# meijieru/AtomNAS

Hardware: AMD Instinct MI355X
Metric: images/sec (whole node) AtomNAS-C supernet 224x224 bs256/GPU (higher is better)
Workload: dtype bf16; 1 GPU; atomnas_c_supernet full training step (fwd + CE-smooth/L2/L1 + bwd + grad all-reduce + RMSprop + EMA), 224x224; per_gpu_batch=256, global_batch=256, parallelism=dp1, hip_graph=True

## Files before the change

### atomnas_amd/csrc/optim.hip

```cpp
#include "common.h"

namespace atomnas {

enum { HYP_LR = 0, HYP_RHO = 1, HYP_EMA_DECAY = 2, HYP_GRAD_SCALE = 3 };

enum { GUARD_OK = 0, GUARD_SCALE = 1, GUARD_NORM = 2, GUARD_COEF = 3, GUARD_SKIPPED = 4, GUARD_CLIPPED = 5 };

template <bool GUARDED>
__global__ __launch_bounds__(256) void k_rmsprop_ema(float* __restrict__ p, const float* __restrict__ g, float* __restrict__ sq,
                                                     float* __restrict__ buf, float* __restrict__ ema,
                                                     const float* __restrict__ wd_chunk, long n, const float* __restrict__ hyper,
                                                     float alpha, float one_minus_alpha, float eps, int eps_inside_sqrt,
                                                     float momentum, float* __restrict__ l2_part, const float* __restrict__ guard) {
#pragma clang fp contract(off)
  __shared__ float s_part[4];
  const float lr = hyper[HYP_LR], d = hyper[HYP_EMA_DECAY], gs = GUARDED ? guard[GUARD_SCALE] : hyper[HYP_GRAD_SCALE];
  const bool dropped = GUARDED && guard[GUARD_OK] == 0.f;
  const long nchunks = (n + 255) / 256;
  float l2acc = 0.f;
  for (long ch = blockIdx.x; ch < nchunks; ch += gridDim.x) {
    const long i = ch * 256 + threadIdx.x;
    if (i >= n) continue;
    const float wd = wd_chunk ? wd_chunk[ch] : 0.f;
    float pv = p[i];
// ... 122 lines not shown
}

constexpr int GUARD_UNROLL = 4;
constexpr int GUARD_SWEEP = 256 * GUARD_UNROLL;
constexpr int GUARD_MAX_BLOCKS = 1024;

__global__ __launch_bounds__(256) void k_grad_sumsq(const float* __restrict__ g, long n, float* __restrict__ part) {
#pragma clang fp contract(off)
  __shared__ float s_part[4];
  const long n4 = n >> 2;
  const f32x4* __restrict__ g4 = reinterpret_cast<const f32x4*>(g);
  float a[GUARD_UNROLL] = {0.f, 0.f, 0.f, 0.f};
  for (long base = (long)blockIdx.x * GUARD_SWEEP + threadIdx.x; base < n4; base += (long)gridDim.x * GUARD_SWEEP) {
    f32x4 v[GUARD_UNROLL];
#pragma unroll
    for (int u = 0; u < GUARD_UNROLL; ++u) {
      const long i = base + u * 256;
      v[u] = i < n4 ? g4[i] : f32x4{0.f, 0.f, 0.f, 0.f};
    }
#pragma unroll
    for (int u = 0; u < GUARD_UNROLL; ++u) a[u] = a[u] + ((v[u][0] * v[u][0] + v[u][1] * v[u][1]) + (v[u][2] * v[u][2] + v[u][3] * v[u][3]));
  }
  float acc = (a[0] + a[1]) + (a[2] + a[3]);
  const long t = n4 * 4 + threadIdx.x;
  if (blockIdx.x == 0 && threadIdx.x < 3 && t < n) acc = acc + g[t] * g[t];
  acc = wave_sum(acc);
  if ((threadIdx.x & 63) == 0) s_part[threadIdx.x >> 6] = acc;
  __syncthreads();
  if (threadIdx.x == 0) part[blockIdx.x] = ((s_part[0] + s_part[1]) + s_part[2]) + s_part[3];
}

__global__ __launch_bounds__(256) void k_guard_verdict(const float* __restrict__ part, int nparts, const float* __restrict__ hyper,
                                                       float max_norm, int skip_nonfinite, float* __restrict__ guard) {
#pragma clang fp contract(off)
  __shared__ float s_t[256];
  float a = 0.f;
  for (int i = threadIdx.x; i < nparts; i += 256) a += part[i];
  s_t[threadIdx.x] = a;
  __syncthreads();
  for (int o = 128; o > 0; o >>= 1) {
    if ((int)threadIdx.x < o) s_t[threadIdx.x] += s_t[threadIdx.x + o];
    __syncthreads();
  }
  if (threadIdx.x == 0) {
    const float sumsq = s_t[0], gs = hyper[HYP_GRAD_SCALE];
    const float norm = sqrtf(sumsq) * gs;
    const bool finite = isfinite(sumsq);
    float coef = 1.f;
    if (max_norm > 0.f && isfinite(max_norm) && isfinite(norm)) {
      const float c = max_norm / (norm + 1e-6f);
      coef = c < 1.f ? c : 1.f;
    }
    const bool ok = finite || !skip_nonfinite;
    guard[GUARD_OK] = ok ? 1.f : 0.f;
    guard[GUARD_SCALE] = gs * coef;
    guard[GUARD_NORM] = norm;
    guard[GUARD_COEF] = coef;
    int* cnt = reinterpret_cast<int*>(guard);
    if (!ok) cnt[GUARD_SKIPPED] = cnt[GUARD_SKIPPED] + 1;
    if (coef < 1.f) cnt[GUARD_CLIPPED] = cnt[GUARD_CLIPPED] + 1;
  }
}

__global__ __launch_bounds__(256) void k_guard_restore(float* __restrict__ dst, const float* __restrict__ src, long n,
                                                       const float* __restrict__ guard, int unconditional) {
  if (!unconditional && guard[GUARD_OK] != 0.f) return;
  const long n4 = n >> 2;
  f32x4* __restrict__ d4 = reinterpret_cast<f32x4*>(dst);
  const f32x4* __restrict__ s4 = reinterpret_cast<const f32x4*>(src);
  for (long i = (long)blockIdx.x * 256 + threadIdx.x; i < n4; i += (long)gridDim.x * 256) d4[i] = s4[i];
  const long t = n4 * 4 + threadIdx.x;
  if (blockIdx.x == 0 && threadIdx.x < 3 && t < n) dst[t] = src[t];
}

__global__ __launch_bounds__(256) void k_add_i64(long* __restrict__ p, long n, long v) {
  for (long i = (long)blockIdx.x * 256 + threadIdx.x; i < n; i += (long)gridDim.x * 256) p[i] += v;
}

struct PackJob {
  long src_off, dst_off;
  int rows, cols, src_ld, dst_ld, c_off, mode;
};

template <typename T>
__global__ __launch_bounds__(256) void k_pack(const float* __restrict__ arena, void* __restrict__ packbuf, const PackJob* __restrict__ jobs) {
  const PackJob jb = jobs[blockIdx.y];
  const long total = (long)jb.rows * jb.cols;
  const float* src = arena + jb.src_off;
  for (long i = (long)blockIdx.x * 256 + threadIdx.x; i < total; i += (long)gridDim.x * 256) {
    const int r = (int)(i / jb.cols), c = (int)(i % jb.cols);
    const float v = src[(long)r * jb.src_ld + c];
    if (jb.mode == 0) reinterpret_cast<T*>(packbuf)[jb.dst_off + (long)r * jb.dst_ld + jb.c_off + c] = from_f32<T>(v);
    else if (jb.mode == 1) reinterpret_cast<T*>(packbuf)[jb.dst_off + (long)(jb.c_off + c) * jb.dst_ld + r] = from_f32<T>(v);
    else reinterpret_cast<float*>(packbuf)[jb.dst_off + (long)c * jb.dst_ld + jb.c_off + r] = v;
  }
}

}

using namespace atomnas;

static int launch_rmsprop(const char* what, float* p, const float* g, float* sq, float* buf, float* ema, const float* wd_chunk, long n,
                          const float* hyper, double alpha, double eps, int eps_inside_sqrt, double momentum, float* l2_value, float* ws,
                          const float* guard, void* stream) {
  ATOMNAS_REQUIRE(p && g && sq && hyper && n > 0, "%s: bad arguments", what);
  ATOMNAS_REQUIRE(!l2_value || (ws && wd_chunk), "%s: the L2 value needs wd_chunk and a 4096-float workspace", what);
  ATOMNAS_REQUIRE(momentum >= 0.0 && alpha >= 0.0 && eps >= 0.0, "%s: bad hyper-parameters", what);
  ATOMNAS_REQUIRE((momentum > 0.0) == (buf != nullptr), "%s: momentum buffer must be given iff momentum > 0", what);
  long blocks = (n + 255) / 256;
  if (blocks > 4096) blocks = 4096;
  hipLaunchKernelGGL(guard ? k_rmsprop_ema<true> : k_rmsprop_ema<false>, dim3((unsigned)blocks), dim3(256), 0, (hipStream_t)stream, p, g, sq,
                     buf, ema, wd_chunk, n, hyper, (float)alpha, (float)(1.0 - alpha), (float)eps, eps_inside_sqrt, (float)momentum,
                     l2_value ? ws : nullptr, guard);
  if (l2_value)
    hipLaunchKernelGGL(k_sum_partials, dim3(1), dim3(256), 0, (hipStream_t)stream, ws, (int)blocks, 1.f, 0, l2_value);
  return check_launch(what);
}

extern "C" int atomnas_fused_rmsprop_ema(float* p, const float* g, float* sq, float* buf, float* ema, const float* wd_chunk, long n,
                                         const float* hyper, double alpha, double eps, int eps_inside_sqrt, double momentum,
                                         float* l2_value, float* ws, void* stream) {
  return launch_rmsprop("fused_rmsprop_ema", p, g, sq, buf, ema, wd_chunk, n, hyper, alpha, eps, eps_inside_sqrt, momentum, l2_value, ws,
                        nullptr, stream);
}

extern "C" int atomnas_fused_rmsprop_ema_guarded(float* p, const float* g, float* sq, float* buf, float* ema, const float* wd_chunk, long n,
                                                 const float* hyper, double alpha, double eps, int eps_inside_sqrt, double momentum,
                                                 float* l2_value, float* ws, const float* guard, void* stream) {
  ATOMNAS_REQUIRE(guard, "fused_rmsprop_ema_guarded: needs the guard vector");
  return launch_rmsprop("fused_rmsprop_ema_guarded", p, g, sq, buf, ema, wd_chunk, n, hyper, alpha, eps, eps_inside_sqrt, momentum, l2_value,
                        ws, guard, stream);
}

static int launch_sgd(const char* what, float* p, const float* g, float* buf, float* ema, const float* wd_chunk, long n, const float* hyper,
                      double momentum, int nesterov, float* l2_value, float* ws, const float* guard, void* stream) {
  ATOMNAS_REQUIRE(p && g && hyper && n > 0, "%s: bad arguments", what);
  ATOMNAS_REQUIRE(!l2_value || (ws && wd_chunk), "%s: the L2 value needs wd_chunk and a 4096-float workspace", what);
  ATOMNAS_REQUIRE(momentum >= 0.0, "%s: bad hyper-parameters", what);
  ATOMNAS_REQUIRE((momentum > 0.0) == (buf != nullptr), "%s: momentum buffer must be given iff momentum > 0", what);
  ATOMNAS_REQUIRE(!nesterov || momentum > 0.0, "%s: Nesterov momentum needs momentum > 0", what);
  long blocks = (n + 255) / 256;
  if (blocks > 4096) blocks = 4096;
  hipLaunchKernelGGL(guard ? k_sgd_ema<true> : k_sgd_ema<false>, dim3((unsigned)blocks), dim3(256), 0, (hipStream_t)stream, p, g, buf, ema,
                     wd_chunk, n, hyper, (float)momentum, nesterov, l2_value ? ws : nullptr, guard);
  if (l2_value)
    hipLaunchKernelGGL(k_sum_partials, dim3(1), dim3(256), 0, (hipStream_t)stream, ws, (int)blocks, 1.f, 0, l2_value);
  return check_launch(what);
}

extern "C" int atomnas_fused_sgd_ema(float* p, const float* g, float* buf, float* ema, const float* wd_chunk, long n, const float* hyper,
                                     double momentum, int nesterov, float* l2_value, float* ws, void* stream) {
  return launch_sgd("fused_sgd_ema", p, g, buf, ema, wd_chunk, n, hyper, momentum, nesterov, l2_value, ws, nullptr, stream);
}

extern "C" int atomnas_fused_sgd_ema_guarded(float* p, const float* g, float* buf, float* ema, const float* wd_chunk, long n,
                                             const float* hyper, double momentum, int nesterov, float* l2_value, float* ws,
                                             const float* guard, void* stream) {
  ATOMNAS_REQUIRE(guard, "fused_sgd_ema_guarded: needs the guard vector");
  return launch_sgd("fused_sgd_ema_guarded", p, g, buf, ema, wd_chunk, n, hyper, momentum, nesterov, l2_value, ws, guard, stream);
}

extern "C" int atomnas_grad_guard_ws_floats() { return GUARD_MAX_BLOCKS; }

extern "C" int atomnas_grad_guard(const float* g, long n, const float* hyper, float max_norm, int skip_nonfinite, float* ws, float* guard,
                                  void* stream) {
  ATOMNAS_REQUIRE(g && hyper && ws && guard && n > 0, "grad_guard: bad arguments");
  ATOMNAS_REQUIRE(((unsigned long long)g & 15ull) == 0, "grad_guard: needs a 16-byte aligned gradient arena");
  ATOMNAS_REQUIRE(!(max_norm != max_norm), "grad_guard: max_norm is NaN");
  long blocks = (n / 4 + GUARD_SWEEP - 1) / GUARD_SWEEP;
  if (blocks > GUARD_MAX_BLOCKS) blocks = GUARD_MAX_BLOCKS;
  if (blocks < 1) blocks = 1;
  hipLaunchKernelGGL(k_grad_sumsq, dim3((unsigned)blocks), dim3(256), 0, (hipStream_t)stream, g, n, ws);
  hipLaunchKernelGGL(k_guard_verdict, dim3(1), dim3(256), 0, (hipStream_t)stream, ws, (int)blocks, hyper, max_norm, skip_nonfinite, guard);
  return check_launch("grad_guard");
}

extern "C" int atomnas_guard_restore(float* dst, const float* src, long n, const float* guard, int unconditional, void* stream) {
  ATOMNAS_REQUIRE(dst && src && n > 0 && (guard || unconditional), "guard_restore: bad arguments");
  ATOMNAS_REQUIRE((((unsigned long long)dst | (unsigned long long)src) & 15ull) == 0, "guard_restore: needs 16-byte aligned pointers");
  long blocks = (n / 4 + 255) / 256;
  if (blocks > 2048) blocks = 2048;
  if (blocks < 1) blocks = 1;
  hipLaunchKernelGGL(k_guard_restore, dim3((unsigned)blocks), dim3(256), 0, (hipStream_t)stream, dst, src, n, guard, unconditional);
  return check_launch("guard_restore");
}

extern "C" int atomnas_vec_sum(const float* x, int n, float scale, float* out, void* stream) {
  ATOMNAS_REQUIRE(x && out && n > 0, "vec_sum: bad arguments");
  hipLaunchKernelGGL(k_sum_partials, dim3(1), dim3(256), 0, (hipStream_t)stream, x, n, scale, 0, out);
  return check_launch("vec_sum");
}

extern "C" int atomnas_ema_update(float* shadow, const float* x, long n, const float* hyper, void* stream) {
  ATOMNAS_REQUIRE(shadow && x && hyper && n > 0, "ema_update: bad arguments");
  long blocks = (n + 255) / 256;
  if (blocks > 2048) blocks = 2048;
  hipLaunchKernelGGL(k_ema<false>, dim3((unsigned)blocks), dim3(256), 0, (hipStream_t)stream, shadow, x, n, hyper, (const float*)nullptr);
  return check_launch("ema_update");
}

extern "C" int atomnas_ema_update_guarded(float* shadow, const float* x, long n, const float* hyper, const float* guard, void* stream) {
  ATOMNAS_REQUIRE(shadow && x && hyper && guard && n > 0, "ema_update_guarded: bad arguments");
  long blocks = (n + 255) / 256;
  if (blocks > 2048) blocks = 2048;
  hipLaunchKernelGGL(k_ema<true>, dim3((unsigned)blocks), dim3(256), 0, (hipStream_t)stream, shadow, x, n, hyper, guard);
  return check_launch("ema_update_guarded");
}

extern "C" int atomnas_scale_by(float* x, long n, const float* hyper, int idx, void* stream) {
  ATOMNAS_REQUIRE(x && hyper && n > 0 && idx >= 0 && idx < 4, "scale_by: bad arguments");
  long blocks = (n + 255) / 256;
  if (blocks > 2048) blocks = 2048;
  hipLaunchKernelGGL(k_scale_by, dim3((unsigned)blocks), dim3(256), 0, (hipStream_t)stream, x, n, hyper, idx);
  return check_launch("scale_by");
}

extern "C" int atomnas_accum_fold(float* acc, float* cur, const float* base, long n, int first, int last, float inv_count, void* stream) {
  ATOMNAS_REQUIRE(acc && cur && n > 0, "accum_fold: bad arguments");
  ATOMNAS_REQUIRE((((unsigned long long)acc | (unsigned long long)cur | (unsigned long long)base) & 15ull) == 0,
                  "accum_fold: needs 16-byte aligned pointers");
  long blocks = (n / 4 + 255) / 256;
  if (blocks > 2048) blocks = 2048;
  if (blocks < 1) blocks = 1;
  hipLaunchKernelGGL(k_accum_fold, dim3((unsigned)blocks), dim3(256), 0, (hipStream_t)stream, acc, cur, base, n, first, last, inv_count);
  return check_launch("accum_fold");
}

extern "C" int atomnas_zero(void* p, long bytes, void* stream) {
  ATOMNAS_REQUIRE(p && bytes > 0 && bytes % 4 == 0 && ((unsigned long long)p & 15ull) == 0, "zero: needs a 16-byte aligned pointer and whole words");
  const long n16 = bytes / 16;
  const int ntail = (int)((bytes % 16) / 4);
  long blocks = (n16 + 255) / 256;
  if (blocks > 4096) blocks = 4096;
  if (blocks < 1) blocks = 1;
  hipLaunchKernelGGL(k_zero, dim3((unsigned)blocks), dim3(256), 0, (hipStream_t)stream, (f32x4*)p, n16, (float*)p + n16 * 4, ntail);
  return check_launch("zero");
}

extern "C" int atomnas_add_i64(long* p, long n, long v, void* stream) {
  ATOMNAS_REQUIRE(p && n > 0, "add_i64: bad arguments");
  long blocks = (n + 255) / 256;
  if (blocks > 1024) blocks = 1024;
  hipLaunchKernelGGL(k_add_i64, dim3((unsigned)blocks), dim3(256), 0, (hipStream_t)stream, p, n, v);
  return check_launch("add_i64");
}

extern "C" int atomnas_pack_weights(const float* arena, void* packbuf, const void* jobs_dev, int njobs, int dtype, void* stream) {
  ATOMNAS_REQUIRE(arena && packbuf && jobs_dev && njobs > 0, "pack_weights: bad arguments");
  dim3 grid(32, njobs);
  hipStream_t st = (hipStream_t)stream;
  if (dtype == DT_F32) hipLaunchKernelGGL(k_pack<float>, grid, dim3(256), 0, st, arena, packbuf, (const PackJob*)jobs_dev);
  else hipLaunchKernelGGL(k_pack<bf16_t>, grid, dim3(256), 0, st, arena, packbuf, (const PackJob*)jobs_dev);
  return check_launch("pack_weights");
}

namespace atomnas {
struct RegJob {
  long off;
  int count;
  float coef;
};

__global__ __launch_bounds__(256) void k_reg_grad(const float* __restrict__ p, float* __restrict__ g, const RegJob* __restrict__ jobs,
                                                  int use_sign, const float* __restrict__ mult_ptr, const float* __restrict__ go_ptr) {
  const RegJob jb = jobs[blockIdx.y];
  float m = jb.coef;
  if (mult_ptr) m *= mult_ptr[0];
  if (go_ptr) m *= go_ptr[0];
  for (int i = blockIdx.x * 256 + threadIdx.x; i < jb.count; i += gridDim.x * 256) {
    const float v = p[jb.off + i];
    const float d = use_sign ? ((v > 0.f) ? 1.f : ((v < 0.f) ? -1.f : 0.f)) : v;
    g[jb.off + i] += m * d;
  }
}

__global__ __launch_bounds__(256) void k_reg_value(const float* __restrict__ p, const RegJob* __restrict__ jobs, int use_abs,
                                                   const float* __restrict__ mult_ptr, float post_scale, float* __restrict__ ws) {
  __shared__ float s_part[4];
  const RegJob jb = jobs[blockIdx.y];
  float acc = 0.f;
  for (int i = blockIdx.x * 256 + threadIdx.x; i < jb.count; i += gridDim.x * 256) {
    const float v = p[jb.off + i];
    acc += use_abs ? fabsf(v) : v * v;
  }
  acc = wave_sum(acc);
  if ((threadIdx.x & 63) == 0) s_part[threadIdx.x >> 6] = acc;
  __syncthreads();
  if (threadIdx.x == 0) {
    float m = jb.coef * post_scale;
    if (mult_ptr) m *= mult_ptr[0];
    ws[blockIdx.y * gridDim.x + blockIdx.x] = m * (((s_part[0] + s_part[1]) + s_part[2]) + s_part[3]);
  }
}

}

extern "C" int atomnas_reg_grad(const float* p, float* g, const void* jobs_dev, int njobs, int use_sign, const float* mult_ptr,
                                const float* grad_out_ptr, void* stream) {
  ATOMNAS_REQUIRE(p && g && jobs_dev && njobs > 0, "reg_grad: bad arguments");
  hipLaunchKernelGGL(atomnas::k_reg_grad, dim3(64, njobs), dim3(256), 0, (hipStream_t)stream, p, g, (const atomnas::RegJob*)jobs_dev,
                     use_sign, mult_ptr, grad_out_ptr);
  return atomnas::check_launch("reg_grad");
}

extern "C" int atomnas_reg_value(const float* p, const void* jobs_dev, int njobs, int use_abs, const float* mult_ptr,
                                 float post_scale, float* out, float* ws, void* stream) {
  ATOMNAS_REQUIRE(p && out && ws && jobs_dev && njobs > 0, "reg_value: bad arguments");
  hipLaunchKernelGGL(atomnas::k_reg_value, dim3(64, njobs), dim3(256), 0, (hipStream_t)stream, p, (const atomnas::RegJob*)jobs_dev,
                     use_abs, mult_ptr, post_scale, ws);
  hipLaunchKernelGGL(atomnas::k_sum_partials, dim3(1), dim3(256), 0, (hipStream_t)stream, ws, 64 * njobs, 1.f, 1, out);
  return atomnas::check_launch("reg_value");
}
```

### atomnas_amd/csrc/pwconv.hip

```cpp
#include "pwconv.h"

namespace atomnas {

template <typename T, int MODE, int NCG>
__global__ __launch_bounds__(256) void k_gemm_nt(Operand A, const T* __restrict__ Wp, int ldw, Epilogue ep, long M, int N, int K,
                                                 int Kpad) {
  using MM = Mma<T>;
  constexpr int E = MM::EPL;
  constexpr int KS = 4 * E;
  constexpr int SWD = 64 * NCG;
  extern __shared__ float s_stat[];

  const int tid = threadIdx.x;
  const int lane = tid & 63;
  const int wave = tid >> 6;
  const int q = lane >> 4, j = lane & 15;
  const int wrow = 16 * (j >> 2) + (j & 3);
  const bool do_stats = ep.stats != nullptr && ep.stat_mode != STAT_NONE;
  float* sw = s_stat + wave * 2 * SWD;

  if (do_stats) {
    for (int i = tid; i < 8 * SWD; i += 256) s_stat[i] = 0.f;
    __syncthreads();
  }
// ... 1881 lines not shown
  auto kern = k_gemm_nt_st<KSTEPS, EPK, Cfg::PD, BT, Cfg::WPE, 0, SH>;
  const size_t lds = (size_t)(SH ? 2 : 4) * BT * KSTEPS * 1024 +
                     (EPK == ST_FWD ? 0 : (size_t)4 * (16 + 64) * PB_RP * sizeof(bf16_t) + 4 * 128 * sizeof(float));
  const long waves = (long)num_cus() * resident_per_cu(kern, 256, lds) * 4;
  const long wchunks = SH ? (long)((nchunks + 3) / 4) * 4 : nchunks;
  long tiles_per_item = st_tiles_per_item(mtiles, wchunks, waves, min_tpi, 0);
  if (tiles_per_item > 4096) tiles_per_item = 4096;
  const long nrg = (mtiles + tiles_per_item - 1) / tiles_per_item;
  const long blocks = SH ? nrg * ((nchunks + 3) / 4) : (nrg * nchunks + 3) / 4;
  hipLaunchKernelGGL(kern, dim3((unsigned)blocks), dim3(256), lds, a.st, a.A, (const bf16_t*)a.Wp, a.ldw, ep, a.M, a.N, a.K, nchunks,
                     (int)tiles_per_item, (float*)nullptr);
  return check_launch("gemm_nt_st");
}
static int nt_st_launch(const NtStPlan& p, const NtArgs& a) {
  auto go = [&](auto ks, auto epk) {
    constexpr int KSTEPS = decltype(ks)::value, EPK = decltype(epk)::value;
    using Cfg = StCfg<KSTEPS, EPK>;
    const int nchunks = (a.N + 63) / 64;
    if (Cfg::SH && ((nchunks + 3) / 4 * 4 - nchunks) * 20 <= nchunks) return nt_st_launch_as<KSTEPS, EPK, Cfg::SH, Cfg::BT>(a);
    return nt_st_launch_as<KSTEPS, EPK, false, Cfg::BTP>(a);
  };
  auto kind = [&](auto ks) { return p.kind == ST_FWD ? go(ks, IC<ST_FWD>{}) : go(ks, IC<ST_MASK>{}); };
  return p.ksteps == 1 ? kind(IC<1>{}) : p.ksteps == 2 ? kind(IC<2>{}) : p.ksteps == 3 ? kind(IC<3>{}) : kind(IC<6>{});
}

struct NtSmallPlan { int kst, ntile; };
constexpr int SMALL_MAXN = 64, SMALL_MAXK = 64;
constexpr long SMALL_MINM = 65536;

static bool nt_small_plan(const NtArgs& a, NtSmallPlan& p) {
  if (a.N > SMALL_MAXN || a.K > SMALL_MAXK || a.M < SMALL_MINM) return false;
  p.kst = a.K <= 32 ? 1 : 2;
  p.ntile = (pw_env().small_narrow && !a.ep.out_f32 && a.N % 4 == 0) ? (a.N <= 16 ? 1 : a.N <= 32 ? 2 : 4) : 0;
  return true;
}
static int nt_small_launch(const NtSmallPlan& p, const NtArgs& a) {
  auto go = [&](auto mode, auto kst) {
    constexpr int MODE = decltype(mode)::value, KST = decltype(kst)::value;
    auto kern = p.ntile == 1 ? k_gemm_nt_small<MODE, KST, 1> : p.ntile == 2 ? k_gemm_nt_small<MODE, KST, 2>
              : p.ntile == 4 ? k_gemm_nt_small<MODE, KST, 4> : k_gemm_nt_small<MODE, KST, 0>;
    const size_t lds = a.stats ? (size_t)8 * 64 * sizeof(float) : 0;
    const long R = row_slots(kern, 256, lds, 1, (a.M + 63) / 64, stat_cap(a));
    hipLaunchKernelGGL(kern, dim3((unsigned)R), dim3(256), lds, a.st, a.A, (const bf16_t*)a.Wp, a.ldw, a.ep, a.M, a.N, a.K);
  };
  for_mode(a.mode, [&](auto mode) { p.kst == 1 ? go(mode, IC<1>{}) : go(mode, IC<2>{}); });
  return check_launch("gemm_nt_small");
}

struct NtWsPlan { int ncg, rt; };
constexpr int WS_MINK = 97;
constexpr long WS_MINM = 4096;
constexpr long WS_RT2_MINM = 100000;

static bool nt_ws_plan(const NtArgs& a, NtWsPlan& p) {
  if (a.K < WS_MINK || a.M < WS_MINM) return false;
  p.ncg = a.N > 64 ? 2 : 1;
  p.rt = (a.mode == PRO_BNBWD && a.M >= WS_RT2_MINM) ? 2 : 1;
  return true;
}
template <int MODE, int NCG, int RT>
static void nt_ws_launch_as(const NtArgs& a) {
  auto kern = k_gemm_nt_ws<MODE, NCG, RT>;
  const int ngroups = (a.N + 64 * NCG - 1) / (64 * NCG);
  const size_t lds = (size_t)2 * 64 * NCG * WS_WP * sizeof(bf16_t) + 2 * 3 * WS_KC * sizeof(float) +
                     (a.stats ? (size_t)8 * 64 * NCG * sizeof(float) : 0);
  const long R = row_slots(kern, 256, lds, ngroups, (a.M + 64 * RT - 1) / (64 * RT), stat_cap(a));
  const int wrows = (a.N + 63) / 64 * 64;
  hipLaunchKernelGGL(kern, dim3((unsigned)(R * ngroups)), dim3(256), lds, a.st, a.A, (const bf16_t*)a.Wp, a.ldw, wrows, a.ep, a.M, a.N, a.K);
}
static int nt_ws_launch(const NtWsPlan& p, const NtArgs& a) {
  for_mode(a.mode, [&](auto mode) {
    constexpr int MODE = decltype(mode)::value;
    if constexpr (MODE == PRO_BNBWD) {
      if (p.rt == 2) return p.ncg == 2 ? nt_ws_launch_as<MODE, 2, 2>(a) : nt_ws_launch_as<MODE, 1, 2>(a);
    }
    return p.ncg == 2 ? nt_ws_launch_as<MODE, 2, 1>(a) : nt_ws_launch_as<MODE, 1, 1>(a);
  });
  return check_launch("gemm_nt_ws");
}

struct NtGenericPlan { int ncg; };
static bool nt_generic_plan(const NtArgs& a, NtGenericPlan& p) {
  p.ncg = a.N > 64 ? 2 : 1;
  return true;
}
template <typename T>
static int nt_generic_launch(const NtGenericPlan& p, const NtArgs& a) {
  constexpr int KS = 4 * Mma<T>::EPL;
  const int Kpad = (a.K + KS - 1) / KS * KS;
  auto go = [&](auto mode, auto ncg) {
    constexpr int NCG = decltype(ncg)::value;
    auto kern = k_gemm_nt<T, decltype(mode)::value, NCG>;
    const int ngroups = (a.N + 64 * NCG - 1) / (64 * NCG);
    const size_t lds = a.stats ? (size_t)8 * 64 * NCG * sizeof(float) : 0;
    const long R = row_slots(kern, 256, lds, ngroups, (a.M + 63) / 64, stat_cap(a));
    hipLaunchKernelGGL(kern, dim3((unsigned)(R * ngroups)), dim3(256), lds, a.st, a.A, (const T*)a.Wp, a.ldw, a.ep, a.M, a.N, a.K, Kpad);
  };
  for_mode(a.mode, [&](auto mode) { p.ncg == 2 ? go(mode, IC<2>{}) : go(mode, IC<1>{}); });
  return check_launch("gemm_nt");
}

template <typename T>
static int launch_nt(const NtArgs& a) {
  if constexpr (sizeof(T) == 2) {
    NtSwPlan sw;
    if (nt_sw_plan(a, sw)) return nt_sw_launch(sw, a);
    NtSwgPlan swg;
    if (nt_swg_plan(a, swg)) return nt_swg_launch(swg, a);
    NtStPlan st;
    if (nt_st_plan(a, st)) return nt_st_launch(st, a);
    NtSmallPlan small;
    if (nt_small_plan(a, small)) return nt_small_launch(small, a);
    NtWsPlan ws;
    if (nt_ws_plan(a, ws)) return nt_ws_launch(ws, a);
  }
  NtGenericPlan g;
  nt_generic_plan(a, g);
  return nt_generic_launch<T>(g, a);
}

static NtArgs project_bwd_args(const void* g, int ldg, const void* wpt, int ldw, const void* z, int ldz, long z_ss, const float* zscale,
                               const float* zshift, int act, void* gh, int ldgh, long gh_ss, float* stats, int stat_rows, long M, int oup,
                               int hid, hipStream_t st) {
  const Operand A{g, ldg, nullptr, 0, 0, 0, nullptr, nullptr, nullptr, 0};
  const Epilogue ep{gh, ldgh, 0, nullptr, 0, z, ldz, gh_ss, z_ss, zscale, zshift, act, nullptr, stats, STAT_Z, stat_rows};
  return nt_args(PRO_NONE, A, wpt, ldw, ep, M, hid, oup, st);
}
template <int KSTEPS, int UT>
static int launch_project_bwd_st(const NtArgs& a, float* dwp, long si, long sj, float* ws, long ws_floats) {
  using Cfg = StCfg<KSTEPS, ST_PBWD>;
  const long M = a.M;
  const int N = a.N, K = a.K;
  const int nchunks = (N + 63) / 64;
  const long mtiles = (M + 15) / 16;
  auto kern = k_gemm_nt_st<KSTEPS, ST_PBWD, Cfg::PD, Cfg::BT, Cfg::WPE, UT, false>;
  const size_t lds = (size_t)4 * Cfg::BT * KSTEPS * 1024 + (size_t)4 * (16 * UT + 64) * PB_RP * sizeof(bf16_t) + 4 * 128 * sizeof(float);
  const long waves = (long)num_cus() * resident_per_cu(kern, 256, lds) * 4;
  const long max_parts = ws_floats / ((long)K * N);
  ATOMNAS_REQUIRE(max_parts >= 1, "project_bwd: workspace too small for one partial (%ld floats)", (long)K * N);
  const long tiles_per_item = st_tiles_per_item(mtiles, nchunks, waves, (mtiles + a.ep.stat_rows - 1) / a.ep.stat_rows, max_parts);
  ATOMNAS_REQUIRE(tiles_per_item <= 4096, "project_bwd: %ld row tiles per work item (workspace / statistics rows too small for M=%ld)", tiles_per_item, M);
  const long nranges = (mtiles + tiles_per_item - 1) / tiles_per_item;
  const long items = nranges * nchunks;
  hipLaunchKernelGGL(kern, dim3((unsigned)((items + 3) / 4)), dim3(256), lds, a.st, a.A, (const bf16_t*)a.Wp, a.ldw, a.ep, M, N, K, nchunks,
                     (int)tiles_per_item, ws);
  if (int rc = check_launch("project_bwd_st")) return rc;
  return reduce_parts(ws, (long)K * N, (int)nranges, (long)K * N, dwp, N, si, sj, a.st);
}

#define XB_INSTANCES(X) X(1, 5) X(1, 7) X(1, 12) X(2, 5) X(2, 7) X(3, 5)
static inline int xb_nch(int HT) {
  const int n = (HT + WS_KC - 1) / WS_KC;
  return n <= 5 ? 5 : (n <= 7 ? 7 : (n <= 12 ? 12 : 0));
}
static bool xb_has_instance(int inp, int hid) {
  const int ut = (inp + 15) / 16, nch = xb_nch(hid);
#define X(UTV, NCHV) if (ut == UTV && nch == NCHV) return true;
  XB_INSTANCES(X)
#undef X
  return false;
}
struct XbArgs {
  const bf16_t* h; int ldh; long hss; const float* c1;
  const bf16_t* x; int ldx; const bf16_t* W; int ldw; const bf16_t* add; int ldadd; bf16_t* gx; int ldgx;
  const bf16_t* mpk; int ldm; const float* vb;
  float *dwe, *ws; long ws_floats; long M; int N, K; hipStream_t st;
// ... 144 lines not shown
```

### atomnas_amd/csrc/pwconv_tn.hip

```cpp
#include "pwconv.h"

namespace atomnas {

constexpr int UT_MAX = 20;
constexpr int TN_ROWS = 32;

template <typename T, int UMODE, int VMODE>
__global__ __launch_bounds__(256) void k_gemm_tn(Operand U, int NU, Operand V, int NV, float* __restrict__ out, long si, long sj,
                                                 long M, long rows_per_block, float* __restrict__ ws) {
  using MM = Mma<T>;
  constexpr int E = MM::EPL;
  constexpr int SUB = TN_ROWS / (4 * E);
  constexpr int UP = 16 * UT_MAX + 2;
  constexpr int VP = 64 + 2;
  __shared__ T s_u[TN_ROWS * UP];
  __shared__ T s_v[TN_ROWS * VP];

  const int tid = threadIdx.x;
  const int lane = tid & 63, wave = tid >> 6;
  const int q = lane >> 4, j = lane & 15;

  const int u0 = blockIdx.z * (16 * UT_MAX);
  const int nu = min(NU - u0, 16 * UT_MAX);
  const int ut = (nu + 15) / 16;
// ... 491 lines not shown
    }
  }
}

struct TnArgs {
  int umode; Operand U; int NU;
  int vmode; Operand V; int NV;
  float* out; long si, sj, M;
  float* ws; long ws_floats;
  hipStream_t st;
};

template <int... Vs, typename F> static int for_value(int v, F&& f) {
  int rc = 1;
  (void)((v == Vs ? (rc = f(IC<Vs>{}), true) : false) || ...);
  return rc;
}
template <typename F> static int for_pair(int umode, int vmode, F&& f) {
#define X(UM, VM) if (umode == UM && vmode == VM) return f(IC<UM>{}, IC<VM>{});
  X(PRO_NONE, PRO_NONE) X(PRO_NONE, PRO_BNBWD) X(PRO_BNBWD, PRO_BNRELU) X(PRO_BNRELU, PRO_BNBWD) X(PRO_BNBWD, PRO_NONE)
  X(PRO_NONE, PRO_BNRELU)
#undef X
  set_error("gemm_tn: unsupported prologue pair (%d,%d)", umode, vmode);
  return 1;
}

static int tn_utt(int NU, bool dma) {
  const int ut = (NU + 15) / 16;
  return ut <= 2 ? (dma ? 4 : 2) : ut <= 4 ? 4 : ut <= 6 ? 6 : ut <= 12 ? 12 : ut <= 20 ? 10 : 20;
}

static long tn_ws_cap(const TnArgs& a) { return a.ws ? a.ws_floats / ((long)a.NU * a.NV) : 1; }
static void tn_split(long M, long want, long min_rows, long quantum, long& chunks, long& rows) {
  if (want < 1) want = 1;
  rows = (M + want - 1) / want;
  if (rows < min_rows) rows = min_rows;
  rows = (rows + quantum - 1) / quantum * quantum;
  chunks = (M + rows - 1) / rows;
}
static int tn_finish(const char* what, const TnArgs& a, long chunks) {
  if (int rc = check_launch(what)) return rc;
  if (chunks > 1) return reduce_parts(a.ws, (long)a.NU * a.NV, (int)chunks, (long)a.NU * a.NV, a.out, a.NV, a.si, a.sj, a.st);
  return 0;
}

using TnDmaKernel = decltype(&k_gemm_tn3<4, false, 4>);
struct TnDmaPlan { TnDmaKernel kern; int utt, vt, uz; size_t lds; long chunks, rows; unsigned grid; };
constexpr int DMA_MINNU = 32, DMA_MINNV = 256;
constexpr long DMA_MINM = 1024, DMA_MINROWS = 128;
constexpr int tn3_depth(int utt) { return 2 * (4 * (8 + utt) * 1024) + 4096 <= 160 * 1024 ? 4 : 3; }
static bool tn_dma_plan(const TnArgs& a, TnDmaPlan& p) {
  static const int on = getenv("ATOMNAS_TN_DMA") ? atoi(getenv("ATOMNAS_TN_DMA")) : 1;
  if (!on || a.umode != PRO_NONE || (a.vmode != PRO_NONE && a.vmode != PRO_BNRELU) || !a.ws) return false;
  if (a.NV < DMA_MINNV || a.NU < DMA_MINNU || a.M < DMA_MINM) return false;
  p.utt = tn_utt(a.NU, true);
  if (for_value<4, 6, 12, 10>(p.utt, [&](auto utt) {
        constexpr int UTT = decltype(utt)::value, DEPTH = tn3_depth(UTT);
        p.kern = a.vmode == PRO_BNRELU ? k_gemm_tn3<UTT, true, DEPTH> : k_gemm_tn3<UTT, false, DEPTH>;
        p.lds = (size_t)DEPTH * (8 + UTT) * 1024;
        return 0;
      }))
    return false;
  if (p.lds > max_lds_bytes()) return false;
  p.vt = (a.NV + 127) / 128, p.uz = (a.NU + 16 * p.utt - 1) / (16 * p.utt);
  const long tiles = (long)p.vt * p.uz;
  long want = (long)num_cus() * resident_per_cu(p.kern, 256, p.lds) / tiles;
  if (want > a.M / DMA_MINROWS) want = a.M / DMA_MINROWS;
  if (want > tn_ws_cap(a)) want = tn_ws_cap(a);
  want = want / 8 * 8;
  if (want < 8) return false;
  tn_split(a.M, want, 0, 32, p.chunks, p.rows);
  p.grid = (unsigned)((p.chunks + 7) / 8 * 8 * tiles);
  return true;
}
static int tn_dma_launch(const TnDmaPlan& p, const TnArgs& a) {
  hipLaunchKernelGGL(p.kern, dim3(p.grid), dim3(256), p.lds, a.st, a.U, a.NU, a.V, a.NV, a.out, a.si, a.sj, a.M, p.rows, (int)p.chunks, p.vt,
                     p.uz, a.ws);
  return tn_finish("gemm_tn3", a, p.chunks);
}

using TnSlabKernel = decltype(&k_gemm_tn2<PRO_NONE, PRO_NONE, 2, 1, 128>);
struct TnSlabPlan { TnSlabKernel kern; int utt, vtt, slab_rows, vt, uz; size_t lds; long chunks, rows; int xcd; unsigned grid; };
constexpr int SLAB_WIDE_MINNV = 256;
static bool tn_slab_plan(const TnArgs& a, TnSlabPlan& p) {
  p.utt = tn_utt(a.NU, false);
  const bool wide = p.utt >= 4 && p.utt <= 12 && a.NV >= SLAB_WIDE_MINNV;
  p.vtt = wide ? 2 : 1, p.slab_rows = wide ? 64 : 128;
  if (for_pair(a.umode, a.vmode, [&](auto um, auto vm) {
        return for_value<2, 4, 6, 12, 10, 20>(p.utt, [&](auto utt) {
          constexpr int UM = decltype(um)::value, VM = decltype(vm)::value, UTT = decltype(utt)::value;
          p.kern = k_gemm_tn2<UM, VM, UTT, 1, 128>;
          if constexpr (UTT >= 4 && UTT <= 12)
            if (wide) p.kern = k_gemm_tn2<UM, VM, UTT, 2, 64>;
          return 0;
        });
      }))
    return false;
  const int vw = 64 * p.vtt, uw = 16 * p.utt;
  p.vt = (a.NV + vw - 1) / vw, p.uz = (a.NU + uw - 1) / uw;
  p.lds = (size_t)(vw + uw) * (p.slab_rows + 8) * sizeof(bf16_t) + (size_t)3 * (vw + uw) * sizeof(float);
  const long tiles = (long)p.vt * p.uz;
  long want = (long)num_cus() * resident_per_cu(p.kern, 256, p.lds) / tiles;
  if (want > a.M / (2 * p.slab_rows)) want = a.M / (2 * p.slab_rows);
  if (want > tn_ws_cap(a)) want = tn_ws_cap(a);
  p.xcd = want >= 8;
  if (p.xcd) want = want / 8 * 8;
  tn_split(a.M, want, 0, 1, p.chunks, p.rows);
  p.grid = (unsigned)((p.xcd ? (p.chunks + 7) / 8 * 8 : p.chunks) * tiles);
  return true;
}
static int tn_slab_launch(const TnSlabPlan& p, const TnArgs& a) {
  hipLaunchKernelGGL(p.kern, dim3(p.grid), dim3(256), p.lds, a.st, a.U, a.NU, a.V, a.NV, a.out, a.si, a.sj, a.M, p.rows, (int)p.chunks, p.vt,
                     p.uz, p.xcd, p.chunks > 1 ? a.ws : nullptr);
  return tn_finish("gemm_tn2", a, p.chunks);
}

using TnGenericKernel = decltype(&k_gemm_tn<float, PRO_NONE, PRO_NONE>);
struct TnGenericPlan { TnGenericKernel kern; int vt, uz; long chunks, rows; };
static bool tn_generic_plan(const TnArgs& a, TnGenericPlan& p) {
  if (for_pair(a.umode, a.vmode, [&](auto um, auto vm) { p.kern = k_gemm_tn<float, decltype(um)::value, decltype(vm)::value>; return 0; }))
    return false;
  p.vt = (a.NV + 63) / 64, p.uz = (a.NU + 16 * UT_MAX - 1) / (16 * UT_MAX);
  const long tiles = (long)p.vt * p.uz;
  long want = (1024 + tiles - 1) / tiles;
  if (want > tn_ws_cap(a)) want = tn_ws_cap(a);
  tn_split(a.M, want, 8 * TN_ROWS, TN_ROWS, p.chunks, p.rows);
  return true;
}
static int tn_generic_launch(const TnGenericPlan& p, const TnArgs& a) {
  hipLaunchKernelGGL(p.kern, dim3((unsigned)p.chunks, p.vt, p.uz), dim3(256), 0, a.st, a.U, a.NU, a.V, a.NV, a.out, a.si, a.sj, a.M, p.rows,
                     p.chunks > 1 ? a.ws : nullptr);
  return tn_finish("gemm_tn", a, p.chunks);
}

static int launch_tn(const TnArgs& a, int dtype) {
  TnDmaPlan dma; TnSlabPlan slab; TnGenericPlan generic;
  if (dtype == DT_BF16 && tn_dma_plan(a, dma)) return tn_dma_launch(dma, a);
  if (dtype == DT_BF16 && tn_slab_plan(a, slab)) return tn_slab_launch(slab, a);
  if (dtype == DT_F32 && tn_generic_plan(a, generic)) return tn_generic_launch(generic, a);
  return 1;
}

}

using namespace atomnas;

extern "C" int atomnas_pw_gemm_tn(int u_mode, const void* u, int ldu, long u_ss, const void* u2, int ldu2, long u2_ss, const float* uc1,
                                  const float* uc2, const float* uc3, int u_relu, int NU, int v_mode, const void* v, int ldv, long v_ss,
                                  const void* v2, int ldv2, long v2_ss, const float* vc1, const float* vc2, const float* vc3, int v_relu, int NV, float* out,
                                  long si, long sj, long M, float* ws, long ws_floats, int dtype, void* stream) {
  ATOMNAS_REQUIRE(dtype == DT_F32 || dtype == DT_BF16, "pw_gemm_tn: bad dtype %d", dtype);
  ATOMNAS_REQUIRE(M > 0 && NU > 0 && NV > 0 && out, "pw_gemm_tn: empty shape");
  Operand U{u, ldu, u2, ldu2, u_ss, u2_ss, uc1, uc2, uc3, u_relu};
  Operand V{v, ldv, v2, ldv2, v_ss, v2_ss, vc1, vc2, vc3, v_relu};
  ATOMNAS_REQUIRE((u_ss == 0 || u_ss >= M * 16) && (v_ss == 0 || v_ss >= M * 16), "pw_gemm_tn: slab stride smaller than M*16");
  if (check_operand("pw_gemm_tn(U)", U, u_mode, NU)) return 1;
  if (check_operand("pw_gemm_tn(V)", V, v_mode, NV)) return 1;
  return launch_tn(TnArgs{u_mode, U, NU, v_mode, V, NV, out, si, sj, M, ws, ws_floats, (hipStream_t)stream}, dtype);
}
```

### atomnas_amd/csrc/reduce.hip

```cpp
#include "common.h"
#include <mutex>
#include <vector>

namespace atomnas {

__global__ __launch_bounds__(256) void k_reduce_parts(const float* __restrict__ part, long part_stride, int parts, long n,
                                                      float* __restrict__ out, int inner, long s_outer, long s_inner) {
  __shared__ float s_acc[8][32];
  const int el = threadIdx.x & 31, pg = threadIdx.x >> 5;
  const long e = (long)blockIdx.x * 32 + el;
  float a0 = 0.f, a1 = 0.f, a2 = 0.f, a3 = 0.f;
  if (e < n) {
    int r = pg;
    for (; r + 24 < parts; r += 32) {
      a0 += part[(long)r * part_stride + e];
      a1 += part[(long)(r + 8) * part_stride + e];
      a2 += part[(long)(r + 16) * part_stride + e];
      a3 += part[(long)(r + 24) * part_stride + e];
    }
    for (; r < parts; r += 8) a0 += part[(long)r * part_stride + e];
  }
  s_acc[pg][el] = (a0 + a1) + (a2 + a3);
  __syncthreads();
  if (pg == 0 && e < n) {
    float t = s_acc[0][el];
#pragma unroll
    for (int g = 1; g < 8; ++g) t += s_acc[g][el];
    const long o = (e / inner) * s_outer + (e % inner) * s_inner;
    out[o] += t;
  }
}

struct ReduceJob {
  const float* part;
  float* out;
  long part_stride, n, s_outer, s_inner;
  int parts, inner;
  unsigned blk0, pad_;
};
constexpr int RJ_MAX = 56;
struct ReduceBatch {
  ReduceJob j[RJ_MAX];
  int njobs;
};

__global__ __launch_bounds__(256) void k_reduce_batch(const ReduceBatch b) {
  __shared__ float s_acc[8][32];
  int ji = 0;
  while (ji + 1 < b.njobs && blockIdx.x >= b.j[ji + 1].blk0) ++ji;
  const ReduceJob& jb = b.j[ji];
  const float* __restrict__ part = jb.part;
  const long part_stride = jb.part_stride, n = jb.n;
  const int parts = jb.parts;
  const int el = threadIdx.x & 31, pg = threadIdx.x >> 5;
  const long e = (long)(blockIdx.x - jb.blk0) * 32 + el;
  float a0 = 0.f, a1 = 0.f, a2 = 0.f, a3 = 0.f;
  if (e < n) {
    int r = pg;
    for (; r + 24 < parts; r += 32) {
      a0 += part[(long)r * part_stride + e];
      a1 += part[(long)(r + 8) * part_stride + e];
      a2 += part[(long)(r + 16) * part_stride + e];
      a3 += part[(long)(r + 24) * part_stride + e];
    }
    for (; r < parts; r += 8) a0 += part[(long)r * part_stride + e];
  }
  s_acc[pg][el] = (a0 + a1) + (a2 + a3);
  __syncthreads();
  if (pg == 0 && e < n) {
    float t = s_acc[0][el];
#pragma unroll
    for (int g = 1; g < 8; ++g) t += s_acc[g][el];
    const long o = (e / jb.inner) * jb.s_outer + (e % jb.inner) * jb.s_inner;
    jb.out[o] += t;
  }
}

static std::mutex g_rj_mu;
static bool g_rj_defer = false;
static hipStream_t g_rj_stream = nullptr;
static std::vector<ReduceJob> g_rj;

static bool rj_conflict(const ReduceJob& a, const ReduceJob& b) {
  auto hi = [](const ReduceJob& j) { return j.out + ((j.n - 1) / j.inner) * j.s_outer + (long)(j.inner - 1) * j.s_inner; };
  if (hi(a) < b.out || hi(b) < a.out) return false;
  if (a.s_inner == 1 && b.s_inner == 1 && a.s_outer == b.s_outer && a.inner <= a.s_outer && b.inner <= b.s_outer) {
    const long d = (b.out - a.out) % a.s_outer;
    const long cb = d < 0 ? d + a.s_outer : d;
    if (cb >= a.inner && cb + b.inner <= a.s_outer) return false;
  }
  return true;
}

static int flush_jobs_locked(hipStream_t st) {
  size_t i = 0;
  while (i < g_rj.size()) {
    ReduceBatch b;
    b.njobs = 0;
    unsigned blk = 0;
    while (i < g_rj.size() && b.njobs < RJ_MAX) {
      bool clash = false;
      for (int q = 0; q < b.njobs && !clash; ++q) clash = rj_conflict(b.j[q], g_rj[i]);
      if (clash) break;
      ReduceJob j = g_rj[i++];
      j.blk0 = blk;
      blk += (unsigned)((j.n + 31) / 32);
      b.j[b.njobs++] = j;
    }
    hipLaunchKernelGGL(k_reduce_batch, dim3(blk), dim3(256), 0, st, b);
  }
  g_rj.clear();
  return check_launch("reduce_flush");
}

int reduce_parts(const float* part, long part_stride, int parts, long n, float* out, int inner, long s_outer, long s_inner,
                 hipStream_t st) {
  if (n <= 0 || parts <= 0) return 0;
  {
    std::lock_guard<std::mutex> lock(g_rj_mu);
    if (g_rj_defer && st == g_rj_stream) {
      g_rj.push_back(ReduceJob{part, out, part_stride, n, s_outer, s_inner, parts, inner, 0u, 0u});
      return 0;
    }
  }
  const long blocks = (n + 31) / 32;
  hipLaunchKernelGGL(k_reduce_parts, dim3((unsigned)blocks), dim3(256), 0, st, part, part_stride, parts, n, out, inner, s_outer,
                     s_inner);
  return check_launch("reduce_parts");
}

}

using namespace atomnas;

extern "C" int atomnas_reduce_defer(int on, void* stream) {
  std::lock_guard<std::mutex> lock(g_rj_mu);
  int rc = 0;
  if (!on && !g_rj.empty()) rc = flush_jobs_locked((hipStream_t)stream);
  g_rj_defer = on != 0;
  g_rj_stream = (hipStream_t)stream;
  return rc;
}

extern "C" int atomnas_reduce_flush(void* stream) {
  std::lock_guard<std::mutex> lock(g_rj_mu);
  if (g_rj.empty()) return 0;
  return flush_jobs_locked((hipStream_t)stream);
}


namespace atomnas {
struct FoldJob {
  float* src;
  float* dst;
  long src_ld, dst_ld;
  int rows, cols;
  unsigned blk0;
  int pad_;
};
static_assert(sizeof(FoldJob) == 48, "atomnas_fold_job layout");

__global__ __launch_bounds__(256) void k_fold_jobs(const FoldJob* __restrict__ jobs, int njobs, unsigned blk_base) {
  const unsigned b = blockIdx.x + blk_base;
  int lo = 0, hi = njobs - 1;
  while (lo < hi) {
    const int mid = (lo + hi + 1) >> 1;
    if (jobs[mid].blk0 <= b) lo = mid; else hi = mid - 1;
  }
  const FoldJob jb = jobs[lo];
  const long e = (long)(b - jb.blk0) * 256 + threadIdx.x;
  if (e >= (long)jb.rows * jb.cols) return;
  const int r = (int)(e / jb.cols), c = (int)(e % jb.cols);
  float* s = jb.src + r * jb.src_ld + c;
  jb.dst[r * jb.dst_ld + c] += *s;
  *s = 0.f;
}
}

extern "C" int atomnas_fold_jobs(const void* jobs_dev, int first, int njobs, long blk_base, long nblocks, void* stream) {
  ATOMNAS_REQUIRE(jobs_dev && first >= 0 && njobs > 0 && blk_base >= 0 && nblocks > 0 && blk_base + nblocks < (1L << 31), "fold_jobs: bad arguments");
  hipLaunchKernelGGL(atomnas::k_fold_jobs, dim3((unsigned)nblocks), dim3(256), 0, (hipStream_t)stream,
                     (const atomnas::FoldJob*)jobs_dev + first, njobs, (unsigned)blk_base);
  return atomnas::check_launch("fold_jobs");
}
```

Before: 9627 images/sec.

## Tile weight packing, vectorize partial reductions, and widen grids for small GEMMs

The weight-pack kernel now works on 64x64 tiles with vectorized 4-wide loads and stores, and transposed modes go through shared memory so global accesses coalesce. The partial-sum reduction handles 128 elements per block using f32x4 loads. The NT GEMM planner falls back to a single column group when two would leave CUs idle, and the TN slab planner tries smaller U tiles for small M to raise block count. These changes target memory-bound auxiliary kernels and under-occupied small GEMMs, at the cost of more code paths and alignment-dependent branches.

```diff
diff --git a/atomnas_amd/csrc/optim.hip b/atomnas_amd/csrc/optim.hip
--- a/atomnas_amd/csrc/optim.hip
+++ b/atomnas_amd/csrc/optim.hip
@@ -228,17 +228,84 @@
   int rows, cols, src_ld, dst_ld, c_off, mode;
 };
 
+constexpr int PACK_TILE = 64;
+constexpr int PACK_GRID_X = 64;
+
+template <typename D>
+__device__ __forceinline__ void pack_store4(D* __restrict__ d, const float (&v)[4], int cnt) {
+  if (cnt == 4 && (reinterpret_cast<uintptr_t>(d) & (4 * sizeof(D) - 1)) == 0) {
+    VecIO<D, 4>::store(d, v);
+  } else {
+#pragma unroll
+    for (int k = 0; k < 4; ++k)
+      if (k < cnt) d[k] = from_f32<D>(v[k]);
+  }
+}
+
+__device__ __forceinline__ void pack_load4(const float* __restrict__ s, float (&v)[4], int cnt) {
+  if (cnt == 4 && (reinterpret_cast<uintptr_t>(s) & 15) == 0) {
+    VecIO<float, 4>::load(s, v);
+  } else {
+#pragma unroll
+    for (int k = 0; k < 4; ++k) v[k] = k < cnt ? s[k] : 0.f;
+  }
+}
+
+template <typename D>
+__device__ __forceinline__ void pack_store_t(D* __restrict__ dst, long dst_ld, const float (*tile)[PACK_TILE + 1], int r0, int c0, int rows,
+                                             int cols) {
+  const int rq = (threadIdx.x & 15) * 4;
+#pragma unroll
+  for (int pass = 0; pass < PACK_TILE / 16; ++pass) {
+    const int cl = pass * 16 + (threadIdx.x >> 4);
+    const int cnt = min(4, rows - (r0 + rq));
+    if (c0 + cl < cols && cnt > 0) {
+      const float v[4] = {tile[rq][cl], tile[rq + 1][cl], tile[rq + 2][cl], tile[rq + 3][cl]};
+      pack_store4<D>(dst + (long)(c0 + cl) * dst_ld + r0 + rq, v, cnt);
+    }
+  }
+}
+
 template <typename T>
 __global__ __launch_bounds__(256) void k_pack(const float* __restrict__ arena, void* __restrict__ packbuf, const PackJob* __restrict__ jobs) {
+  __shared__ float tile[PACK_TILE][PACK_TILE + 1];
   const PackJob jb = jobs[blockIdx.y];
-  const long total = (long)jb.rows * jb.cols;
-  const float* src = arena + jb.src_off;
-  for (long i = (long)blockIdx.x * 256 + threadIdx.x; i < total; i += (long)gridDim.x * 256) {
-    const int r = (int)(i / jb.cols), c = (int)(i % jb.cols);
-    const float v = src[(long)r * jb.src_ld + c];
-    if (jb.mode == 0) reinterpret_cast<T*>(packbuf)[jb.dst_off + (long)r * jb.dst_ld + jb.c_off + c] = from_f32<T>(v);
-    else if (jb.mode == 1) reinterpret_cast<T*>(packbuf)[jb.dst_off + (long)(jb.c_off + c) * jb.dst_ld + r] = from_f32<T>(v);
-    else reinterpret_cast<float*>(packbuf)[jb.dst_off + (long)c * jb.dst_ld + jb.c_off + r] = v;
+  const float* __restrict__ src = arena + jb.src_off;
+  const int tc = (jb.cols + PACK_TILE - 1) / PACK_TILE;
+  const int ntiles = ((jb.rows + PACK_TILE - 1) / PACK_TILE) * tc;
+  const int cq = (threadIdx.x & 15) * 4, rl = threadIdx.x >> 4;
+  for (int t = blockIdx.x; t < ntiles; t += gridDim.x) {
+    const int r0 = (t / tc) * PACK_TILE, c0 = (t % tc) * PACK_TILE;
+    const int cnt = min(4, jb.cols - (c0 + cq));
+    if (jb.mode == 0) {
+      T* __restrict__ dst = reinterpret_cast<T*>(packbuf) + jb.dst_off + jb.c_off;
+#pragma unroll
+      for (int pass = 0; pass < PACK_TILE / 16; ++pass) {
+        const int r = r0 + pass * 16 + rl;
+        if (r < jb.rows && cnt > 0) {
+          float v[4];
+          pack_load4(src + (long)r * jb.src_ld + c0 + cq, v, cnt);
+          pack_store4<T>(dst + (long)r * jb.dst_ld + c0 + cq, v, cnt);
+        }
+      }
+      continue;
+    }
+    __syncthreads();
+#pragma unroll
+    for (int pass = 0; pass < PACK_TILE / 16; ++pass) {
+      const int rt = pass * 16 + rl;
+      if (r0 + rt < jb.rows && cnt > 0) {
+        float v[4];
+        pack_load4(src + (long)(r0 + rt) * jb.src_ld + c0 + cq, v, cnt);
+#pragma unroll
+        for (int k = 0; k < 4; ++k) tile[rt][cq + k] = v[k];
+      }
+    }
+    __syncthreads();
+    if (jb.mode == 1)
+      pack_store_t<T>(reinterpret_cast<T*>(packbuf) + jb.dst_off + (long)jb.c_off * jb.dst_ld, jb.dst_ld, tile, r0, c0, jb.rows, jb.cols);
+    else
+      pack_store_t<float>(reinterpret_cast<float*>(packbuf) + jb.dst_off + jb.c_off, jb.dst_ld, tile, r0, c0, jb.rows, jb.cols);
   }
 }
 
@@ -393,7 +460,7 @@
 
 extern "C" int atomnas_pack_weights(const float* arena, void* packbuf, const void* jobs_dev, int njobs, int dtype, void* stream) {
   ATOMNAS_REQUIRE(arena && packbuf && jobs_dev && njobs > 0, "pack_weights: bad arguments");
-  dim3 grid(32, njobs);
+  dim3 grid(PACK_GRID_X, njobs);
   hipStream_t st = (hipStream_t)stream;
   if (dtype == DT_F32) hipLaunchKernelGGL(k_pack<float>, grid, dim3(256), 0, st, arena, packbuf, (const PackJob*)jobs_dev);
   else hipLaunchKernelGGL(k_pack<bf16_t>, grid, dim3(256), 0, st, arena, packbuf, (const PackJob*)jobs_dev);
diff --git a/atomnas_amd/csrc/pwconv.hip b/atomnas_amd/csrc/pwconv.hip
--- a/atomnas_amd/csrc/pwconv.hip
+++ b/atomnas_amd/csrc/pwconv.hip
@@ -1987,6 +1987,7 @@
 struct NtGenericPlan { int ncg; };
 static bool nt_generic_plan(const NtArgs& a, NtGenericPlan& p) {
   p.ncg = a.N > 64 ? 2 : 1;
+  if (p.ncg == 2 && (a.M + 63) / 64 * ((a.N + 127) / 128) < num_cus()) p.ncg = 1;
   return true;
 }
 template <typename T>
diff --git a/atomnas_amd/csrc/pwconv_tn.hip b/atomnas_amd/csrc/pwconv_tn.hip
--- a/atomnas_amd/csrc/pwconv_tn.hip
+++ b/atomnas_amd/csrc/pwconv_tn.hip
@@ -597,9 +597,9 @@
 using TnSlabKernel = decltype(&k_gemm_tn2<PRO_NONE, PRO_NONE, 2, 1, 128>);
 struct TnSlabPlan { TnSlabKernel kern; int utt, vtt, slab_rows, vt, uz; size_t lds; long chunks, rows; int xcd; unsigned grid; };
 constexpr int SLAB_WIDE_MINNV = 256;
-static bool tn_slab_plan(const TnArgs& a, TnSlabPlan& p) {
-  p.utt = tn_utt(a.NU, false);
-  const bool wide = p.utt >= 4 && p.utt <= 12 && a.NV >= SLAB_WIDE_MINNV;
+static bool tn_slab_plan_as(const TnArgs& a, TnSlabPlan& p, int utt, bool allow_wide) {
+  p.utt = utt;
+  const bool wide = allow_wide && p.utt >= 4 && p.utt <= 12 && a.NV >= SLAB_WIDE_MINNV;
   p.vtt = wide ? 2 : 1, p.slab_rows = wide ? 64 : 128;
   if (for_pair(a.umode, a.vmode, [&](auto um, auto vm) {
         return for_value<2, 4, 6, 12, 10, 20>(p.utt, [&](auto utt) {
@@ -624,6 +624,16 @@
   p.grid = (unsigned)((p.xcd ? (p.chunks + 7) / 8 * 8 : p.chunks) * tiles);
   return true;
 }
+constexpr long SLAB_SMALL_M = 4 * 128;
+static bool tn_slab_plan(const TnArgs& a, TnSlabPlan& p) {
+  if (!tn_slab_plan_as(a, p, tn_utt(a.NU, false), true)) return false;
+  if (a.M >= SLAB_SMALL_M || p.chunks != 1) return true;
+  for (int utt : {12, 10, 6, 4, 2}) {
+    if ((long)p.vt * p.uz >= num_cus()) break;
+    if (utt < p.utt) tn_slab_plan_as(a, p, utt, false);
+  }
+  return true;
+}
 static int tn_slab_launch(const TnSlabPlan& p, const TnArgs& a) {
   hipLaunchKernelGGL(p.kern, dim3(p.grid), dim3(256), p.lds, a.st, a.U, a.NU, a.V, a.NV, a.out, a.si, a.sj, a.M, p.rows, (int)p.chunks, p.vt,
                      p.uz, p.xcd, p.chunks > 1 ? a.ws : nullptr);
diff --git a/atomnas_amd/csrc/reduce.hip b/atomnas_amd/csrc/reduce.hip
--- a/atomnas_amd/csrc/reduce.hip
+++ b/atomnas_amd/csrc/reduce.hip
@@ -4,31 +4,54 @@
 
 namespace atomnas {
 
+constexpr int RED_EPB = 128;
+
+__device__ __forceinline__ void reduce_block(const float* __restrict__ part, long part_stride, int parts, long n, long e0,
+                                             float* __restrict__ out, int inner, long s_outer, long s_inner, float (*s_acc)[RED_EPB]) {
+  const int ln = threadIdx.x & 31, pg = threadIdx.x >> 5;
+  const long e = e0 + ln * 4;
+  f32x4 a0 = {0.f, 0.f, 0.f, 0.f}, a1 = a0, a2 = a0, a3 = a0;
+  if (e + 3 < n && (part_stride & 3) == 0 && (reinterpret_cast<uintptr_t>(part + e) & 15) == 0) {
+    const float* __restrict__ q = part + e;
+    int r = pg;
+    for (; r + 24 < parts; r += 32) {
+      a0 += *reinterpret_cast<const f32x4*>(q + (long)r * part_stride);
+      a1 += *reinterpret_cast<const f32x4*>(q + (long)(r + 8) * part_stride);
+      a2 += *reinterpret_cast<const f32x4*>(q + (long)(r + 16) * part_stride);
+      a3 += *reinterpret_cast<const f32x4*>(q + (long)(r + 24) * part_stride);
+    }
+    for (; r < parts; r += 8) a0 += *reinterpret_cast<const f32x4*>(q + (long)r * part_stride);
+  } else {
+#pragma unroll
+    for (int k = 0; k < 4; ++k) {
+      if (e + k >= n) break;
+      const float* __restrict__ q = part + e + k;
+      int r = pg;
+      for (; r + 24 < parts; r += 32) {
+        a0[k] += q[(long)r * part_stride];
+        a1[k] += q[(long)(r + 8) * part_stride];
+        a2[k] += q[(long)(r + 16) * part_stride];
+        a3[k] += q[(long)(r + 24) * part_stride];
+      }
+      for (; r < parts; r += 8) a0[k] += q[(long)r * part_stride];
+    }
+  }
+  *reinterpret_cast<f32x4*>(&s_acc[pg][ln * 4]) = (a0 + a1) + (a2 + a3);
+  __syncthreads();
+  const long eo = e0 + threadIdx.x;
+  if (threadIdx.x < RED_EPB && eo < n) {
+    float t = s_acc[0][threadIdx.x];
+#pragma unroll
+    for (int g = 1; g < 8; ++g) t += s_acc[g][threadIdx.x];
+    const long o = (eo / inner) * s_outer + (eo % inner) * s_inner;
+    out[o] += t;
+  }
+}
+
 __global__ __launch_bounds__(256) void k_reduce_parts(const float* __restrict__ part, long part_stride, int parts, long n,
                                                       float* __restrict__ out, int inner, long s_outer, long s_inner) {
-  __shared__ float s_acc[8][32];
-  const int el = threadIdx.x & 31, pg = threadIdx.x >> 5;
-  const long e = (long)blockIdx.x * 32 + el;
-  float a0 = 0.f, a1 = 0.f, a2 = 0.f, a3 = 0.f;
-  if (e < n) {
-    int r = pg;
-    for (; r + 24 < parts; r += 32) {
-      a0 += part[(long)r * part_stride + e];
-      a1 += part[(long)(r + 8) * part_stride + e];
-      a2 += part[(long)(r + 16) * part_stride + e];
-      a3 += part[(long)(r + 24) * part_stride + e];
-    }
-    for (; r < parts; r += 8) a0 += part[(long)r * part_stride + e];
-  }
-  s_acc[pg][el] = (a0 + a1) + (a2 + a3);
-  __syncthreads();
-  if (pg == 0 && e < n) {
-    float t = s_acc[0][el];
-#pragma unroll
-    for (int g = 1; g < 8; ++g) t += s_acc[g][el];
-    const long o = (e / inner) * s_outer + (e % inner) * s_inner;
-    out[o] += t;
-  }
+  __shared__ __attribute__((aligned(16))) float s_acc[8][RED_EPB];
+  reduce_block(part, part_stride, parts, n, (long)blockIdx.x * RED_EPB, out, inner, s_outer, s_inner, s_acc);
 }
 
 struct ReduceJob {
@@ -45,35 +68,12 @@
 };
 
 __global__ __launch_bounds__(256) void k_reduce_batch(const ReduceBatch b) {
-  __shared__ float s_acc[8][32];
+  __shared__ __attribute__((aligned(16))) float s_acc[8][RED_EPB];
   int ji = 0;
   while (ji + 1 < b.njobs && blockIdx.x >= b.j[ji + 1].blk0) ++ji;
   const ReduceJob& jb = b.j[ji];
-  const float* __restrict__ part = jb.part;
-  const long part_stride = jb.part_stride, n = jb.n;
-  const int parts = jb.parts;
-  const int el = threadIdx.x & 31, pg = threadIdx.x >> 5;
-  const long e = (long)(blockIdx.x - jb.blk0) * 32 + el;
-  float a0 = 0.f, a1 = 0.f, a2 = 0.f, a3 = 0.f;
-  if (e < n) {
-    int r = pg;
-    for (; r + 24 < parts; r += 32) {
-      a0 += part[(long)r * part_stride + e];
-      a1 += part[(long)(r + 8) * part_stride + e];
-      a2 += part[(long)(r + 16) * part_stride + e];
-      a3 += part[(long)(r + 24) * part_stride + e];
-    }
-    for (; r < parts; r += 8) a0 += part[(long)r * part_stride + e];
-  }
-  s_acc[pg][el] = (a0 + a1) + (a2 + a3);
-  __syncthreads();
-  if (pg == 0 && e < n) {
-    float t = s_acc[0][el];
-#pragma unroll
-    for (int g = 1; g < 8; ++g) t += s_acc[g][el];
-    const long o = (e / jb.inner) * jb.s_outer + (e % jb.inner) * jb.s_inner;
-    jb.out[o] += t;
-  }
+  reduce_block(jb.part, jb.part_stride, jb.parts, jb.n, (long)(blockIdx.x - jb.blk0) * RED_EPB, jb.out, jb.inner, jb.s_outer, jb.s_inner,
+               s_acc);
 }
 
 static std::mutex g_rj_mu;
@@ -104,7 +104,7 @@
       if (clash) break;
       ReduceJob j = g_rj[i++];
       j.blk0 = blk;
-      blk += (unsigned)((j.n + 31) / 32);
+      blk += (unsigned)((j.n + RED_EPB - 1) / RED_EPB);
       b.j[b.njobs++] = j;
     }
     hipLaunchKernelGGL(k_reduce_batch, dim3(blk), dim3(256), 0, st, b);
@@ -123,7 +123,7 @@
       return 0;
     }
   }
-  const long blocks = (n + 31) / 32;
+  const long blocks = (n + RED_EPB - 1) / RED_EPB;
   hipLaunchKernelGGL(k_reduce_parts, dim3((unsigned)blocks), dim3(256), 0, st, part, part_stride, parts, n, out, inner, s_outer,
                      s_inner);
   return check_launch("reduce_parts");
```

Measured after the change: 9758 images/sec, median of 6. 1.4% higher.
